# feldroop/genedex

Hardware: NVIDIA B200
Metric: len-50 count queries/s on 3.1 Gbp DNA index (locate: see `locate`) (higher is better)
Workload: dtype u64

## Files before the change

genedex_b200/_lib.py:

```python
from __future__ import annotations

import ctypes as C
import os

_HERE = os.path.dirname(os.path.abspath(__file__))
LIB_PATH = os.environ.get("GENEDEX_B200_LIB") or os.path.join(_HERE, "csrc", "libgenedex_b200.so")

GDX_OK, GDX_ERR_INVALID_SYMBOL, GDX_ERR_BAD_ARG, GDX_ERR_CUDA, GDX_ERR_OOM, GDX_ERR_TEXT_TOO_LONG, \
    GDX_ERR_UNSUPPORTED, GDX_ERR_BUSY = range(8)
GDX_I32, GDX_U32, GDX_I64 = 0, 1, 2
GDX_CONSTRUCT_HOST, GDX_CONSTRUCT_DEVICE, GDX_CONSTRUCT_AUTO = 0, 1, 2
GDX_FLAG_VERIFY_SUFFIX_ARRAY = 1
GDX_FLAG_NO_TEXT = 2
GDX_FLAG_NO_INVERSE_SAMPLES = 4
GDX_FLAG_NO_DENSE_SUFFIX_ARRAY = 8
GDX_FLAG_NO_SEED_TABLE = 16
GDX_FLAG_NO_ROW_CONTEXT_TABLE = 32
GDX_QUERIES_IO_BYTES, GDX_QUERIES_PACKED_2BIT = 0, 1
GDX_RANK_CONDENSED, GDX_RANK_FLAT = 0, 1
GDX_NCCL_UNIQUE_ID_BYTES = 128
GDX_ABI_VERSION = 2
GDX_HAMMING_MAX_MISMATCHES = 3
GDX_HAMMING_MAX_QUERY_LEN = 256

# ... 33 lines not shown
                ("lookup_table_depth", C.c_uint32), ("sampled_suffix_array_u32", C.c_void_p),
                ("flags", C.c_uint32), ("accelerator_budget_bytes", C.c_uint64),
                ("rank_variant", C.c_uint32), ("block_bits", C.c_uint32)]


class gdx_index_info(C.Structure):
    _fields_ = [("text_len", C.c_uint64), ("num_texts", C.c_uint64), ("num_dense_symbols", C.c_uint32),
                ("num_searchable_dense_symbols", C.c_uint32), ("storage", C.c_uint32),
                ("sampling_rate", C.c_uint32), ("lookup_table_depth", C.c_uint32), ("rank_layout", C.c_uint32),
                ("rank_record_bytes", C.c_uint32), ("rank_positions_per_record", C.c_uint32),
                ("device", C.c_int32), ("image_bytes", C.c_uint64), ("rank_bytes", C.c_uint64),
                ("sample_bytes", C.c_uint64), ("lookup_bytes", C.c_uint64), ("num_samples", C.c_uint64),
                ("num_text_borders", C.c_uint64), ("text_bytes", C.c_uint64),
                ("inverse_sample_bytes", C.c_uint64), ("dense_suffix_array_bytes", C.c_uint64), ("seed_table_bytes", C.c_uint64),
                ("seed_table_depth", C.c_uint32), ("row_context_entry_bytes", C.c_uint32)]


class gdx_stats(C.Structure):
    _fields_ = [("queries", C.c_uint64), ("lf_steps", C.c_uint64), ("hits", C.c_uint64),
                ("walk_steps", C.c_uint64), ("kernel_ms_search", C.c_double),
                ("kernel_ms_locate", C.c_double), ("kernel_launches", C.c_uint64),
                ("verified_queries", C.c_uint64), ("locate_walk_steps", C.c_uint64),
                ("packed_queries", C.c_uint64), ("exception_queries", C.c_uint64), ("h2d_bytes", C.c_uint64),
                ("d2h_bytes", C.c_uint64), ("shards", C.c_uint64)]


_vp, _u64, _i32, _u32 = C.c_void_p, C.c_uint64, C.c_int32, C.c_uint32
_P = C.POINTER
PROTOTYPES = {
    "gdx_abi_version": (_u32, []),
    "gdx_last_error_message": (C.c_char_p, []),
    "gdx_last_error_query": (_u64, []),
    "gdx_device_count": (_i32, []),
    "gdx_index_build": (C.c_int, [_vp, _vp, _u64, _P(gdx_alphabet), _P(gdx_config), _P(_vp)]),
    "gdx_index_create_from_parts": (C.c_int, [_P(gdx_parts), _i32, _P(_vp)]),
    "gdx_index_create_from_bwt": (C.c_int, [_vp, _P(gdx_parts), _i32, _P(_vp)]),
    "gdx_suffix_array": (C.c_int, [_vp, _u64, _u32, _u32, _i32, _vp]),
    "gdx_concat_texts": (C.c_int, [_vp, _vp, _u64, _P(gdx_alphabet), _vp, _vp, _vp]),
    "gdx_index_download_bwt": (C.c_int, [_vp, _vp]),
    "gdx_index_get_count": (C.c_int, [_vp, _vp]),
    "gdx_index_download_samples": (C.c_int, [_vp, _vp]),
    "gdx_index_download_text_borders": (C.c_int, [_vp, _vp, _vp]),
    "gdx_index_destroy": (None, [_vp]),
    "gdx_index_get_info": (C.c_int, [_vp, _P(gdx_index_info)]),
    "gdx_index_set_dense_suffix_array": (C.c_int, [_vp, C.c_int32]),
    "gdx_index_set_seed_table_depth": (C.c_int, [_vp, C.c_int32]),
    "gdx_index_set_text_verification": (C.c_int, [_vp, C.c_int32]),
# ... 63 lines not shown
```

genedex_b200/csrc/api.cu:

```cuda
#include <cuda_runtime.h>
#include <dlfcn.h>
#include <type_traits>

#include <algorithm>
#include <atomic>
#include <chrono>
#include <condition_variable>
#include <cstddef>
#include <deque>
#include <thread>
#include <cstdarg>
#include <cstdio>
#include <cstdlib>
#include <cstring>
#include <memory>
#include <mutex>
#include <shared_mutex>
#include <new>
#include <numeric>
#include <string>
#include <utility>
#include <vector>

#include <cub/device/device_radix_sort.cuh>
// ... 600 lines not shown
    if (cudaMalloc(&d, bytes) != cudaSuccess) {
        cudaGetLastError();
        return fail(GDX_ERR_OOM, "row context table: %llu bytes of device memory not available", (unsigned long long)bytes);
    }
    gdx_status st = dispatch_layout(idx->h.layout, [&](auto L) -> gdx_status {
        k_build_row_context<decltype(L)><<<(unsigned)div_up(n, 256), 256>>>(idx->dev, reinterpret_cast<uint4 *>(d), n);
        return GDX_OK;
    });
    cudaError_t e = st == GDX_OK ? cudaDeviceSynchronize() : cudaSuccess;
    if (st != GDX_OK || e != cudaSuccess) {
        cudaFree(d);
        return st != GDX_OK ? st : fail(GDX_ERR_CUDA, "row context table: %s", cudaGetErrorString(e));
    }
    idx->row_ctx = d;
    idx->row_ctx_bytes = bytes;
    idx->dev.row_context = d;
    return GDX_OK;
}

void drop_seed_table(gdx_index *idx) {
    if (!idx->seed_lut) return;
    idx->dev.seed_lookup = nullptr;
    idx->dev.seed_depth = 0;
    cudaFree(idx->seed_lut);
    idx->seed_lut = nullptr;
    idx->seed_lut_bytes = 0;
}

uint64_t seed_entries(uint32_t ns, uint32_t d) {
    uint64_t e = 1;
    for (uint32_t i = 0; i < d; ++i) {
        e *= ns;
        if (e > (1ull << 36)) return 0;
    }
    return e;
}

gdx_status build_seed_table(gdx_index *idx, uint32_t depth) {
    drop_seed_table(idx);
    const ImageHeader &h = idx->h;
    if (depth <= h.lookup_depth || h.n == 0 || h.ns == 0) return GDX_OK;
    const uint64_t esz = h.wide ? 16 : 8, last = seed_entries(h.ns, depth), prev = seed_entries(h.ns, depth - 1);
    if (last == 0 || depth > 40) return fail(GDX_ERR_UNSUPPORTED, "seed table of depth %u is too large", depth);
    void *fin = nullptr, *tmp = nullptr;
    if (cudaMalloc(&fin, last * esz) != cudaSuccess || cudaMalloc(&tmp, prev * esz) != cudaSuccess) {
        cudaGetLastError();
        if (fin) cudaFree(fin);
        return fail(GDX_ERR_OOM, "seed table of depth %u: %llu bytes of device memory not available", depth,
                    (unsigned long long)((last + prev) * esz));
    }
    void *cur = (depth % 2 == 0) ? fin : tmp;
    cudaError_t e;
    if (h.wide) {
        const uint64_t e0[2] = {0, h.n};
        e = cudaMemcpy(cur, e0, sizeof e0, cudaMemcpyHostToDevice);
    } else {
        const uint32_t e0[2] = {0, (uint32_t)h.n};
        e = cudaMemcpy(cur, e0, sizeof e0, cudaMemcpyHostToDevice);
    }
    gdx_status st = GDX_OK;
    for (uint32_t d = 1; d <= depth && e == cudaSuccess && st == GDX_OK; ++d) {
        void *nxt = cur == fin ? tmp : fin;
        const uint64_t entries = seed_entries(h.ns, d);
        st = dispatch_layout(h.layout, [&](auto L) -> gdx_status {
            k_lut_extend<decltype(L)><<<(unsigned)div_up(entries, 256), 256>>>(idx->dev, cur, nxt, entries);
            return GDX_OK;
        });
        e = cudaGetLastError();
        cur = nxt;
    }
    if (e == cudaSuccess && st == GDX_OK) e = cudaDeviceSynchronize();
    cudaFree(tmp);
    if (st != GDX_OK || e != cudaSuccess || cur != fin) {
        cudaFree(fin);
        return st != GDX_OK ? st : fail(GDX_ERR_CUDA, "seed table: %s", cudaGetErrorString(e));
    }
    idx->seed_lut = fin;
    idx->seed_lut_bytes = last * esz;
    idx->dev.seed_lookup = fin;
    idx->dev.seed_depth = depth;
    return GDX_OK;
}

uint64_t accel_room(const gdx_index *idx) {
    if (idx->h.accel_budget) {
        const uint64_t used = idx->dense_sa_bytes + idx->seed_lut_bytes + idx->row_ctx_bytes;
        return idx->h.accel_budget > used ? idx->h.accel_budget - used : 0;
    }
    size_t free_b = 0, total_b = 0;
    if (cudaMemGetInfo(&free_b, &total_b) != cudaSuccess) return 0;
    return free_b / 4;
}

void auto_seed_table(gdx_index *idx) {
    if (!idx || idx->h.n == 0 || idx->h.ns < 2) return;
    const char *e = getenv("GDX_SEED_TABLE");
    uint32_t depth = 0;
    if (e) {
        if (atoi(e) <= 0) return;
        depth = (uint32_t)atoi(e);
    } else {
        if (idx->h.accel_flags & kAccelNoSeedTable) return;
        while (seed_entries(idx->h.ns, depth + 1) && seed_entries(idx->h.ns, depth + 1) <= 4 * idx->h.n) ++depth;
        const uint64_t esz = idx->h.wide ? 16 : 8, room = accel_room(idx);
        size_t free_b = 0, total_b = 0;
        if (cudaMemGetInfo(&free_b, &total_b) != cudaSuccess) return;
        while (depth > 0 && (seed_entries(idx->h.ns, depth) * esz > room ||
                             (seed_entries(idx->h.ns, depth) + seed_entries(idx->h.ns, depth - 1)) * esz > free_b))
            --depth;
    }
    if (depth <= idx->h.lookup_depth) return;
    if (build_seed_table(idx, depth) != GDX_OK) t_error.clear();
}

void auto_dense_sa(gdx_index *idx) {
    if (!idx || idx->h.n == 0) return;
    const char *e = getenv("GDX_DENSE_SA");
    if (e && atoi(e) == 0) return;
    if (!(e && atoi(e) != 0)) {
        if (idx->h.accel_flags & kAccelNoDenseSA) return;
        if (idx->h.n * (idx->h.wide ? 8ull : 4ull) > accel_room(idx)) return;
    }
    if (build_dense_sa(idx) != GDX_OK) t_error.clear();
}

void auto_row_context(gdx_index *idx) {
    if (!idx || !row_context_possible(idx)) return;
    const char *e = getenv("GDX_ROW_CONTEXT");
    if (e && atoi(e) == 0) return;
    if (!(e && atoi(e) != 0)) {
        if (idx->h.accel_flags & kAccelNoRowContext) return;
        const uint64_t room = idx->h.accel_budget ? accel_room(idx) : 2 * accel_room(idx);
        if (idx->h.n * 16 > room) return;
    }
    if (build_row_context(idx) != GDX_OK) t_error.clear();
}

gdx_status build_image(const ImageSources &src, int device, gdx_index **out) {
    std::unique_ptr<gdx_index> idx(new gdx_index());
    GDX_TRY(plan_header(src, idx->h));
    ImageHeader &h = idx->h;
    idx->device = device;
    CUDA_TRY(cudaMalloc(&idx->image, h.image_bytes));
    idx->own_image = true;
    auto cleanup = [&](gdx_status st) {
        cudaFree(idx->image);
        idx->image = nullptr;
        return st;
    };
#define IMG_TRY(expr)                                                                             \
    do {                                                                                          \
        cudaError_t _e = (expr);                                                                  \
        if (_e != cudaSuccess)                                                                    \
            return cleanup(fail(GDX_ERR_CUDA, "%s failed: %s (%s:%d)", #expr,                     \
                                cudaGetErrorString(_e), __FILE__, __LINE__));                     \
    } while (0)
    uint8_t *base = (uint8_t *)idx->image;
    IMG_TRY(cudaMemset(base, 0, h.image_bytes));
// ... 232 lines not shown
        }
    
        if (construction == GDX_CONSTRUCT_DEVICE) {
            DeviceBuildResult r;
            const bool verify = (config->flags & GDX_FLAG_VERIFY_SUFFIX_ARRAY) != 0;
            st = device_build_from_text(nullptr, d_text.p, n, alphabet->num_dense_symbols,
                                        config->suffix_array_sampling_rate, r, t_error, false, verify, keep_isa);
            if (st != GDX_OK) return st;
            if (verify && r.verify_violations) {
                r.release();
                return fail(GDX_ERR_CUDA, "device suffix array failed verification (%llu violations)",
                            (unsigned long long)r.verify_violations);
            }
            src.border_rows = r.border_rows.data();
            src.border_pos = r.border_pos.data();
            src.n_border = r.border_rows.size();
            src.d_bwt = r.d_bwt;
            src.d_samples = r.d_samples;
            src.d_samples_wide = false;
            src.d_isa32 = r.d_isa_samples;
            st = build_image(src, device, out);
            r.release();
            if (st == GDX_OK) {
                auto_dense_sa(*out);
                auto_seed_table(*out);
                auto_row_context(*out);
            }
            return st;
        }
    
        HostParts hp;
        host_parts_from_text(ct.text.data(), n, alphabet->num_dense_symbols, config->suffix_array_sampling_rate, hp);
        uint8_t *d_bwt = nullptr;
        CUDA_TRY(cudaMalloc(&d_bwt, n ? n : 1));
        cudaError_t e = cudaMemcpy(d_bwt, hp.bwt.data(), n, cudaMemcpyHostToDevice);
        if (e != cudaSuccess) {
            cudaFree(d_bwt);
            return fail(GDX_ERR_CUDA, "BWT upload failed: %s", cudaGetErrorString(e));
        }
        src.border_rows = hp.border_rows.data();
        src.border_pos = hp.border_pos.data();
        src.n_border = hp.border_rows.size();
        src.d_bwt = d_bwt;
        src.h_samples64 = hp.samples.data();
        if (keep_isa) src.h_isa64 = hp.isa_samples.data();
        st = build_image(src, device, out);
        cudaFree(d_bwt);
        if (st == GDX_OK) {
            auto_dense_sa(*out);
            auto_seed_table(*out);
            auto_row_context(*out);
        }
        return st;
    });
}

static gdx_status sources_from_parts(const gdx_parts *parts, ImageSources &src,
                                     std::vector<uint64_t> &rows, std::vector<uint64_t> &pos) {
    if (!parts) return fail(GDX_ERR_BAD_ARG, "parts is NULL");
    GDX_TRY(validate_alphabet(parts->alphabet));
    if (parts->sampling_rate == 0) return fail(GDX_ERR_BAD_ARG, "sampling rate must be > 0");
    if (!parts->count || !parts->sentinel_indices || parts->num_texts == 0)
        return fail(GDX_ERR_BAD_ARG, "count / sentinel_indices missing");
    if (parts->text_len > storage_max(parts->storage)) return fail(GDX_ERR_TEXT_TOO_LONG, "text too long for storage");
    std::vector<std::pair<uint64_t, uint64_t>> b(parts->num_text_borders);
    for (uint64_t i = 0; i < parts->num_text_borders; ++i)
        b[i] = {parts->text_border_rows[i], parts->text_border_positions[i]};
    std::sort(b.begin(), b.end());
    rows.resize(b.size());
    pos.resize(b.size());
    for (size_t i = 0; i < b.size(); ++i) {
        rows[i] = b[i].first;
        pos[i] = b[i].second;
    }
// ... 20 lines not shown
extern "C" gdx_status gdx_index_create_from_bwt(const uint8_t *bwt, const gdx_parts *parts, int32_t device_req,
                                                gdx_index **out) {
    return guarded([&]() -> gdx_status {
        if (!out) return fail(GDX_ERR_BAD_ARG, "out is NULL");
        *out = nullptr;
        if (!bwt) return fail(GDX_ERR_BAD_ARG, "bwt is NULL");
        ImageSources src;
        std::vector<uint64_t> rows, pos;
        GDX_TRY(sources_from_parts(parts, src, rows, pos));
        int device;
        GDX_TRY(resolve_device(device_req, &device));
        DeviceGuard guard(device);
        uint8_t *d_bwt = nullptr;
        CUDA_TRY(cudaMalloc(&d_bwt, src.n ? src.n : 1));
        cudaError_t e = cudaMemcpy(d_bwt, bwt, src.n, cudaMemcpyHostToDevice);
        if (e != cudaSuccess) {
            cudaFree(d_bwt);
            return fail(GDX_ERR_CUDA, "BWT upload failed: %s", cudaGetErrorString(e));
        }
        src.d_bwt = d_bwt;
        gdx_status st = build_image(src, device, out);
        cudaFree(d_bwt);
        if (st == GDX_OK) {
            auto_dense_sa(*out);
            auto_seed_table(*out);
            auto_row_context(*out);
        }
        return st;
    });
}

extern "C" gdx_status gdx_index_create_from_parts(const gdx_parts *parts, int32_t device_req, gdx_index **out) {
    return guarded([&]() -> gdx_status {
        if (!out) return fail(GDX_ERR_BAD_ARG, "out is NULL");
        *out = nullptr;
        ImageSources src;
        std::vector<uint64_t> rows, pos;
        GDX_TRY(sources_from_parts(parts, src, rows, pos));
        if (!parts->interleaved_blocks) return fail(GDX_ERR_BAD_ARG, "interleaved_blocks is NULL");
        int device;
        GDX_TRY(resolve_device(device_req, &device));
        DeviceGuard guard(device);
        const uint32_t block_bits = parts->block_bits ? parts->block_bits : 64;
        if ((block_bits != 64 && block_bits != 512) || parts->rank_variant > GDX_RANK_FLAT)
            return fail(GDX_ERR_BAD_ARG, "rank_variant must be GDX_RANK_CONDENSED or GDX_RANK_FLAT, block_bits 64 or 512");
        const bool flat = parts->rank_variant == GDX_RANK_FLAT;
        const uint32_t words = block_bits / 64, used = block_bits - (flat ? 16 : 0);
        const uint32_t units = flat ? parts->alphabet.num_dense_symbols : choose_layout(parts->alphabet.num_dense_symbols).planes;
        const uint64_t nwords = div_up(src.n + 1, used) * units * words;
        uint64_t *d_blocks = nullptr;
        uint8_t *d_bwt = nullptr;
        CUDA_TRY(cudaMalloc(&d_blocks, nwords * 8));
        cudaError_t e = cudaMalloc(&d_bwt, src.n ? src.n : 1);
        if (e == cudaSuccess) e = cudaMemcpy(d_blocks, parts->interleaved_blocks, nwords * 8, cudaMemcpyHostToDevice);
        if (e == cudaSuccess && src.n) {
            k_ref_blocks_to_bwt<<<(unsigned)div_up(src.n, 256), 256>>>(d_blocks, flat ? 1u : 0u, words, units, src.n, d_bwt);
            e = cudaGetLastError();
        }
        cudaFree(d_blocks);
        if (e != cudaSuccess) {
            if (d_bwt) cudaFree(d_bwt);
            return fail(GDX_ERR_CUDA, "block upload failed: %s", cudaGetErrorString(e));
        }
        src.d_bwt = d_bwt;
        gdx_status st = build_image(src, device, out);
        cudaFree(d_bwt);
        if (st == GDX_OK) {
            auto_dense_sa(*out);
            auto_seed_table(*out);
            auto_row_context(*out);
        }
        return st;
    });
}

extern "C" gdx_status gdx_concat_texts(const uint8_t *texts, const uint64_t *text_offsets, uint64_t num_texts,
                                       const gdx_alphabet *alphabet, uint8_t *dense_out, uint64_t *sentinels_out,
                                       uint64_t *count_out) {
    return guarded([&]() -> gdx_status {
        if (!text_offsets || !alphabet || !dense_out || !sentinels_out || !count_out || num_texts == 0)
            return fail(GDX_ERR_BAD_ARG, "NULL argument or no texts");
        GDX_TRY(check_text_offsets(text_offsets, num_texts));
        GDX_TRY(validate_alphabet(*alphabet));
        ConcatText ct;
        uint64_t bad = 0;
        gdx_status st = concat_texts(texts, text_offsets, num_texts, *alphabet, ct, &bad);
        if (st != GDX_OK) {
            t_error_query = bad;
            return fail(st, "text %llu contains a symbol that is not in the alphabet (alphabet.rs:195-198)",
                        (unsigned long long)bad);
        }
        memcpy(dense_out, ct.text.data(), ct.text.size());
        memcpy(sentinels_out, ct.sentinels.data(), ct.sentinels.size() * 8);
// ... 240 lines not shown
                                            int32_t own_image, gdx_index **out) {
    return guarded([&]() -> gdx_status {
        if (!header || !device_image || !out) return fail(GDX_ERR_BAD_ARG, "NULL argument");
        *out = nullptr;
        ImageHeader h;
        memcpy(&h, header, sizeof h);
        GDX_TRY(validate_header(h));
        int device;
        GDX_TRY(resolve_device(device_req, &device));
        gdx_index *idx = new (std::nothrow) gdx_index();
        if (!idx) return fail(GDX_ERR_OOM, "out of host memory");
        idx->h = h;
        idx->image = device_image;
        idx->own_image = own_image != 0;
        idx->device = device;
        idx->dev = make_dev_index(h, device_image);
        {
            DeviceGuard guard(device);
            gdx_status st = init_policies(idx);
            if (st != GDX_OK) {
                delete idx;
                return st;
            }
            auto_dense_sa(idx);
            auto_seed_table(idx);
            auto_row_context(idx);
        }
        *out = idx;
        return GDX_OK;
    });
}

extern "C" gdx_status gdx_index_set_seed_table_depth(gdx_index *idx, int32_t depth) {
    return guarded([&]() -> gdx_status {
        if (!idx) return fail(GDX_ERR_BAD_ARG, "NULL argument");
        std::unique_lock<std::shared_mutex> cfg(idx->cfg_mu, std::try_to_lock);
        if (!cfg.owns_lock()) return fail(GDX_ERR_BUSY, "queries are running on this index: the seed table cannot change now");
        DeviceGuard guard(idx->device);
        if (depth <= 0) {
            drop_seed_table(idx);
            return GDX_OK;
        }
        return build_seed_table(idx, (uint32_t)depth);
    });
}

extern "C" gdx_status gdx_index_set_row_context_table(gdx_index *idx, int32_t on) {
    return guarded([&]() -> gdx_status {
        if (!idx) return fail(GDX_ERR_BAD_ARG, "NULL argument");
        std::unique_lock<std::shared_mutex> cfg(idx->cfg_mu, std::try_to_lock);
        if (!cfg.owns_lock()) return fail(GDX_ERR_BUSY, "queries are running on this index: the row context table cannot change now");
        DeviceGuard guard(idx->device);
        if (on) return build_row_context(idx);
        drop_row_context(idx);
        return GDX_OK;
    });
}

extern "C" gdx_status gdx_index_set_text_verification(gdx_index *idx, int32_t on) {
    return guarded([&]() -> gdx_status {
        if (!idx) return fail(GDX_ERR_BAD_ARG, "NULL argument");
        std::unique_lock<std::shared_mutex> cfg(idx->cfg_mu, std::try_to_lock);
        if (!cfg.owns_lock()) return fail(GDX_ERR_BUSY, "queries are running on this index");
        idx->verify = on != 0;
        return GDX_OK;
    });
// ... 760 lines not shown
        CUDA_TRY(cudaEventRecord(sl.ev_h2d, sl.stream));
        sl.h2d_pending = true;
    }
    return GDX_OK;
}

gdx_status search_result(Workspace *ws, const gdx_stats &io) {
    CUDA_TRY(ws->read_counters(ws->slot[0].stream));
    CUDA_TRY(cudaStreamSynchronize(ws->slot[0].stream));
    const Counters &cnt = *ws->cnt_h;
    t_stats.queries = io.queries;
    t_stats.packed_queries = io.packed_queries;
    t_stats.exception_queries = io.exception_queries;
    t_stats.h2d_bytes = io.h2d_bytes;
    t_stats.d2h_bytes += io.d2h_bytes;
    for (const Slot &s : ws->slot) {
        t_stats.kernel_ms_search += s.timing.elapsed_ms();
        t_stats.kernel_ms_locate += s.locate.timing.elapsed_ms();
    }
    t_stats.lf_steps = cnt.search.lf_steps;
    t_stats.walk_steps = cnt.search.verify_walk_steps + cnt.locate_walk_steps;
    t_stats.locate_walk_steps = cnt.locate_walk_steps;
    t_stats.verified_queries = cnt.search.verified_rows;
    return kernel_error(*std::min_element(cnt.err, cnt.err + kSlots),
                        "symbol in io representation should be valid (alphabet.rs:195-198)");
}

template <class Sink>
gdx_status search_host(const gdx_index *idx, Workspace *ws, const gdx_queries *qs, Sink &sink) {
    const uint64_t nq = qs->nq;
    CUDA_TRY(ws->reset_counters(ws->slot[0].stream));
    CUDA_TRY(cudaEventRecord(ws->ev_a, ws->slot[0].stream));
    for (int s = 1; s < kSlots; ++s) CUDA_TRY(cudaStreamWaitEvent(ws->slot[s].stream, ws->ev_a, 0));
    Trace trace;
    const bool prepacked = qs->encoding == GDX_QUERIES_PACKED_2BIT;
    const uint64_t total_syms = query_bytes_end(qs, nq) - query_bytes_end(qs, 0);
    const uint64_t total_in = prepacked ? (total_syms + 3) / 4 : total_syms;
    const bool pack = nq && !prepacked && idx->pack.usable && pack_enabled() && total_in >= kPackMinBytes;
    const bool src_pinned = nq && is_pinned(qs->bytes);
    Staging u{nq && total_in >= kStageMinBytes && !src_pinned,
              nq && qs->offsets && nq * 8 >= kStageMinBytes && !is_pinned(qs->offsets),
              qs->offsets && nq * 8 >= kStageMinBytes && narrow_enabled()};
    gdx::ChunkPlan plan{qs->offsets, qs->fixed_len, qs->first_symbol, nq, prepacked, pack, pack && src_pinned,
                        kChunkFirst, kChunkMax, kChunkTail, kChunkMaxQueries, 4.0e6 * HostPool::get().threads()};
    LinkQueue link;
    for (Slot &sl : ws->slot) sl.h2d_pending = false;
// ... 338 lines not shown
        HostPool::t_caller_helps = helps;
    };
    std::vector<std::thread> threads;
    threads.reserve(n_local);
    uint32_t started = 1;
    try {
        for (; started < n_local; ++started) threads.emplace_back(run, started);
    } catch (const std::exception &) {
    }
    run(0);
    for (uint32_t k = started; k < n_local; ++k) run(k);
    for (auto &t : threads) t.join();
    gdx_stats sum = {};
    gdx_status st = GDX_OK;
    for (uint32_t k = 0; k < n_local; ++k) {
        const gdx_stats &x = res[k].stats;
        sum.queries += x.queries;
        sum.lf_steps += x.lf_steps;
        sum.hits += x.hits;
        sum.walk_steps += x.walk_steps;
        sum.locate_walk_steps += x.locate_walk_steps;
        sum.kernel_launches += x.kernel_launches;
        sum.verified_queries += x.verified_queries;
        sum.packed_queries += x.packed_queries;
        sum.exception_queries += x.exception_queries;
        sum.h2d_bytes += x.h2d_bytes;
        sum.d2h_bytes += x.d2h_bytes;
        sum.kernel_ms_search = std::max(sum.kernel_ms_search, x.kernel_ms_search);
        sum.kernel_ms_locate = std::max(sum.kernel_ms_locate, x.kernel_ms_locate);
        if (st == GDX_OK && res[k].st != GDX_OK) {
            st = res[k].st;
            t_error = res[k].error;
            t_error_query = res[k].error_query;
        }
    }
    sum.shards = n_local;
    t_stats = sum;
    return st;
}

}

extern "C" gdx_status gdx_count_many_sharded(gdx_index *const *replicas, uint32_t n_local, uint32_t first_shard,
                                             uint32_t n_shards, const gdx_queries *queries, uint64_t *counts) {
    return guarded([&] {
        return run_sharded(replicas, n_local, first_shard, n_shards, queries, [&](uint32_t k, uint64_t b, uint64_t e) {
// ... 600 lines not shown
```

genedex_b200/csrc/device_index.h:

```cpp
#ifndef GDX_DEVICE_INDEX_H
#define GDX_DEVICE_INDEX_H

#include <stdint.h>

#include "rank_core.h"

namespace gdx {

constexpr uint64_t kImageMagic = 0x3130305842584447ull;
constexpr uint32_t kMaxLookupDepth = 24;
constexpr uint32_t kAccelNoDenseSA = 1, kAccelNoSeedTable = 2, kAccelNoRowContext = 4;

struct ImageHeader {
    uint64_t magic;
    uint32_t version;
    uint32_t wide;
    uint64_t n;
    uint64_t ntexts;
    uint64_t n_border;
    uint64_t n_samples;
    uint64_t n_records;
    uint64_t n_superblocks;
    uint32_t sigma, ns, storage, sampling_rate, lookup_depth;
    uint32_t accel_flags;
// ... 11 lines not shown
};

struct DevIndex {
    const uint8_t *records;
    const uint64_t *sbc;
    const void *samples;
    const void *lookup;
    const uint64_t *border_rows;
    const uint64_t *border_pos;
    const uint64_t *sentinels;
    const uint64_t *count;
    const uint8_t *text;
    const void *isa;
    const void *seed_lookup;
    const void *row_context;
    uint64_t n, ntexts, n_border;
    uint32_t sigma, ns, sampling_rate, lookup_depth;
    uint32_t wide, noff, stride, derived_symbol;
    uint32_t sampling_shift;
    uint32_t text_bits;
    uint32_t verify_min_remaining;
    uint32_t isa_rate;
    uint32_t seed_depth;
    uint64_t lut_level_off[kMaxLookupDepth + 1];
    uint64_t lut_pow[kMaxLookupDepth + 1];
    uint8_t io_to_dense[256];
};

inline DevIndex make_dev_index(const ImageHeader &h, const void *image) {
    const uint8_t *base = (const uint8_t *)image;
    DevIndex d;
    d.records = base + h.off_records;
    d.sbc = (const uint64_t *)(base + h.off_sbc);
    d.samples = base + h.off_samples;
    d.lookup = base + h.off_lookup;
    d.border_rows = (const uint64_t *)(base + h.off_border_rows);
    d.border_pos = (const uint64_t *)(base + h.off_border_pos);
    d.sentinels = (const uint64_t *)(base + h.off_sentinels);
    d.count = (const uint64_t *)(base + h.off_count);
    d.text = h.text_bits ? base + h.off_text : nullptr;
    d.text_bits = h.text_bits;
    d.isa = h.has_isa ? base + h.off_isa : nullptr;
    d.n = h.n;
    d.ntexts = h.ntexts;
    d.n_border = h.n_border;
    d.sigma = h.sigma;
    d.ns = h.ns;
    d.sampling_rate = h.sampling_rate;
    d.lookup_depth = h.lookup_depth;
    d.wide = h.wide;
    d.noff = h.layout.noff;
    d.stride = h.layout.stride;
    d.derived_symbol = h.layout.derived_symbol;
    d.sampling_shift = 0xffffffffu;
    d.verify_min_remaining = 8;
    d.isa_rate = h.sampling_rate;
    d.seed_lookup = nullptr;
    d.seed_depth = 0;
    d.row_context = nullptr;
    if ((h.sampling_rate & (h.sampling_rate - 1)) == 0) {
        uint32_t s = 0;
        while ((1u << s) < h.sampling_rate) ++s;
        d.sampling_shift = s;
    }
    for (uint32_t i = 0; i <= kMaxLookupDepth; ++i) {
        d.lut_level_off[i] = h.lut_level_off[i];
        d.lut_pow[i] = h.lut_pow[i];
    }
    for (int i = 0; i < 256; ++i) d.io_to_dense[i] = h.io_to_dense[i];
    return d;
}

}
#endif
```

genedex_b200/csrc/kernels.cuh:

```cuda
#ifndef GDX_KERNELS_CUH
#define GDX_KERNELS_CUH

#include <cuda_runtime.h>
#include <stdint.h>

#include <cub/block/block_scan.cuh>

#include "device_index.h"
#include "hamming.h"
#include "row_context.h"

namespace gdx {

struct DevQueries {
    const uint8_t *bytes;
    const uint64_t *offsets;
    const uint32_t *offsets32;
    uint64_t fixed_len;
    uint64_t nq;
    uint64_t base;
    uint64_t shift;
    const uint32_t *packed;
    uint64_t limit;
};
// ... 230 lines not shown
        const uint64_t ns = bs + L::local_rank(rs, c, s);
        e = bs + L::local_rank(rs, c, e);
        s = ns;
        return;
    }
    typename L::Rec re = L::load(ix, e, c);
    const uint64_t be = sbc_load(ix, e, c);
    s = bs + L::local_rank(rs, c, s);
    e = be + L::local_rank(re, c, e);
}

__device__ __forceinline__ void lut_load(const DevIndex &ix, uint64_t entry, uint64_t &s, uint64_t &e) {
    if (ix.wide) {
        ulonglong2 v = __ldg(reinterpret_cast<const ulonglong2 *>(ix.lookup) + entry);
        s = v.x;
        e = v.y;
    } else {
        uint2 v = __ldg(reinterpret_cast<const uint2 *>(ix.lookup) + entry);
        s = v.x;
        e = v.y;
    }
}

__device__ __forceinline__ void seed_load(const DevIndex &ix, uint64_t entry, uint64_t &s, uint64_t &e) {
    if (ix.wide) {
        const ulonglong2 v = __ldg(reinterpret_cast<const ulonglong2 *>(ix.seed_lookup) + entry);
        s = v.x;
        e = v.y;
    } else {
        const uint2 v = __ldg(reinterpret_cast<const uint2 *>(ix.seed_lookup) + entry);
        s = v.x;
        e = v.y;
    }
}

__device__ __forceinline__ void report_error(uint64_t *err, uint64_t q) {
    if (err) atomicMin(reinterpret_cast<unsigned long long *>(err), (unsigned long long)q);
}

template <class L>
__device__ __forceinline__ uint64_t resolve_row(const DevIndex &ix, uint64_t i, uint32_t &steps) {
    for (;;) {
        const bool sampled = ix.sampling_shift != 0xffffffffu ? (i & ((1ull << ix.sampling_shift) - 1)) == 0
                                                              : (i % ix.sampling_rate) == 0;
        if (sampled) {
            const uint64_t k = ix.sampling_shift != 0xffffffffu ? i >> ix.sampling_shift : i / ix.sampling_rate;
            if (ix.wide) return __ldg(reinterpret_cast<const uint64_t *>(ix.samples) + k) + steps;
            const uint32_t *sp = reinterpret_cast<const uint32_t *>(ix.samples) + k;
// ... 161 lines not shown
    }
    return key;
}

__global__ void __launch_bounds__(256)
k_query_keys(const __grid_constant__ DevIndex ix, const DevQueries qs, uint32_t key_bits, uint32_t key_syms,
             uint32_t *__restrict__ keys, uint32_t *__restrict__ idx) {
    const uint64_t q = (uint64_t)blockIdx.x * blockDim.x + threadIdx.x;
    if (q >= qs.nq) return;
    keys[q] = query_sort_key(ix, qs, q, key_bits, key_syms);
    idx[q] = (uint32_t)q;
}

constexpr uint32_t kQueryStage = 64;
constexpr uint32_t kQuerySlotWords = kQueryStage / 4 + 1;

constexpr int kModeNarrow = 8;
constexpr uint64_t kBadOffsetFlag = 1ull << 62;

struct SearchCounters {
    unsigned long long lf_steps;
    unsigned long long verify_walk_steps;
    unsigned long long verified_rows;
};

template <class L, bool VERIFY, bool CURSORS, bool PACKED>
__global__ void __launch_bounds__(256, VERIFY ? L::kVerifyMinBlocks : L::kSearchMinBlocks)
k_search(const __grid_constant__ DevIndex ix, const DevQueries qs, uint64_t *__restrict__ out_a,
         uint64_t *__restrict__ out_b, int mode_flags, uint64_t q_index_base, uint64_t *err,
         SearchCounters *stats, const uint32_t *__restrict__ perm,
         const uint32_t *__restrict__ slot_map) {
    constexpr uint32_t kTabBytes = PACKED ? 4 : 256;
    constexpr uint32_t kStageWords = PACKED ? 1 : 256 * kQuerySlotWords;
    __shared__ uint8_t tab[kTabBytes];
    __shared__ uint16_t tab2[PACKED ? 2 : 256];
    __shared__ uint32_t stage[kStageWords];
    if constexpr (!PACKED) {
        for (int i = threadIdx.x; i < 256; i += blockDim.x) {
            const uint32_t d = ix.io_to_dense[i];
            tab[i] = (uint8_t)d;
            tab2[i] = ctx_tab2_entry(d, ix.ns);
        }
        __syncthreads();
    }
    const int mode = mode_flags & 7;
    const bool narrow = (mode_flags & kModeNarrow) != 0;
// ... 46 lines not shown
        };
        auto lookup_index = [&](uint64_t p0, uint32_t d, bool &ok) -> uint64_t {
            if (coded && ix.ns == 4 && d <= 32 && p0 >= tail_begin)
                return d ? tail_bits(ptail, (uint32_t)(p0 - tail_begin), d) : 0ull;
            uint64_t li = 0, f = 1;
            for (uint32_t j = 0; j < d; ++j) {
                const uint32_t c = symbol_at(p0 + j);
                if (c == 0 || c > ix.ns) ok = false;
                li += (uint64_t)(c - 1) * f;
                f *= ix.ns;
            }
            return li;
        };

        const uint32_t depth = len < ix.lookup_depth ? (uint32_t)len : ix.lookup_depth;
        uint64_t pos = len - depth;
        uint64_t s = 0, e = 0;
        bool seeded = false;
        if (!bad && ix.seed_lookup && len >= ix.seed_depth) {
            const uint64_t p0 = len - ix.seed_depth;
            bool ok = true;
            const uint64_t li = lookup_index(p0, ix.seed_depth, ok);
            if (ok) {
                seed_load(ix, li, s, e);
                pos = p0;
                seeded = true;
            }
        }
        if (!seeded) {
            bool ok = true;
            const uint64_t li = lookup_index(pos, depth, ok);
            bad = bad || !ok || broken;
            if (!bad) lut_load(ix, ix.lut_level_off[depth] + li, s, e);
        }

        bool direct = false;
        while (!bad && pos > 0 && s != e) {
            if (VERIFY && e - s == 1 && pos >= ix.verify_min_remaining &&
                (!CURSORS || len - pos >= ix.isa_rate)) {
                uint64_t at;
                vrows = 1;
                uint64_t jm = 0;
                uint32_t cm = 0;
                int cmp = -1;
                if (!CURSORS && ix.row_context) {
                    CtxEntry en;
                    {
                        uint64_t e0, e1;
                        ldg128_na(reinterpret_cast<const uint4 *>(ix.row_context) + s, e0, e1);
                        en = CtxEntry{(uint32_t)e0, (uint32_t)(e0 >> 32), (uint32_t)e1, (uint32_t)(e1 >> 32)};
                    }
                    at = en.x;
                    if (coded && tail_begin == 0 && pos <= ctx_valid_len(en))
                        cmp = ctx_matches(en, (uint32_t)pos, ptail.lo, ptail.hi) ? 0 : 1;
                } else {
                    at = resolve_row<L>(ix, s, vsteps);
                }
                if (cmp >= 0) {
                } else if constexpr (PACKED) {
                    cmp = ix.text_bits == 4
                              ? compare_with_text<4, false>(ix, PackedQueryWords<4>{ptail, qs.packed, begin, tail_begin}, pos, at, jm, cm)
                              : compare_with_text<8, false>(ix, PackedQueryWords<8>{ptail, qs.packed, begin, tail_begin}, pos, at, jm, cm);
                } else {
                    cmp = ix.text_bits == 4
// ... 41 lines not shown
            if (mode == 0) {
                a32[slot_q] = (uint32_t)s;
                b32[slot_q] = (uint32_t)e;
            } else {
                a32[slot_q] = (uint32_t)(e - s);
            }
        } else if (mode == 0) {
            out_a[slot_q] = s;
            out_b[slot_q] = e;
        } else if (mode == 1) {
            out_a[slot_q] = e - s;
        } else {
            out_a[slot_q] = s;
            out_b[slot_q] = direct ? kDirectHit : e;
        }
    }
    if (stats) {
        uint32_t tot = __reduce_add_sync(0xffffffffu, steps);
        if ((threadIdx.x & 31) == 0 && tot) atomicAdd(&stats->lf_steps, (unsigned long long)tot);
        if (VERIFY) {
            tot = __reduce_add_sync(0xffffffffu, vsteps);
            if ((threadIdx.x & 31) == 0 && tot) atomicAdd(&stats->verify_walk_steps, (unsigned long long)tot);
            tot = __reduce_add_sync(0xffffffffu, vrows);
            if ((threadIdx.x & 31) == 0 && tot) atomicAdd(&stats->verified_rows, (unsigned long long)tot);
        }
    }
}

template <class L>
__global__ void __launch_bounds__(256)
k_extend(const __grid_constant__ DevIndex ix, uint64_t *__restrict__ starts, uint64_t *__restrict__ ends,
         const uint8_t *__restrict__ io_symbols, uint64_t n, uint64_t *err, uint64_t index_base) {
    const uint64_t q = (uint64_t)blockIdx.x * blockDim.x + threadIdx.x;
    if (q >= n) return;
    uint32_t c = ix.io_to_dense[io_symbols[q]];
    if (c == 0) {
        report_error(err, index_base + q);
        return;
    }
    uint64_t s = starts[q], e = ends[q];
    if (s > ix.n || e > ix.n) {
        report_error(err + 1, index_base + q);
        return;
    }
    if (s != e) {
        lf_pair<L>(ix, c, s, e);
        starts[q] = s;
// ... 361 lines not shown
        sbc[sb * noff + c] = acc;
        acc += t;
    }
}

template <class L>
__global__ void __launch_bounds__(256)
k_lut_fill(const __grid_constant__ DevIndex ix, void *__restrict__ lookup, uint32_t d) {
    const uint64_t i = (uint64_t)blockIdx.x * blockDim.x + threadIdx.x;
    if (i >= ix.lut_pow[d]) return;
    uint64_t s, e;
    lut_load(ix, ix.lut_level_off[d - 1] + i / ix.ns, s, e);
    const uint32_t c = (uint32_t)(i % ix.ns) + 1;
    if (s != e) lf_pair<L>(ix, c, s, e);
    const uint64_t entry = ix.lut_level_off[d] + i;
    if (ix.wide)
        reinterpret_cast<ulonglong2 *>(lookup)[entry] = make_ulonglong2(s, e);
    else
        reinterpret_cast<uint2 *>(lookup)[entry] = make_uint2((uint32_t)s, (uint32_t)e);
}

template <class L>
__global__ void __launch_bounds__(256)
k_lut_extend(const __grid_constant__ DevIndex ix, const void *__restrict__ prev, void *__restrict__ out, uint64_t entries) {
    const uint64_t i = (uint64_t)blockIdx.x * blockDim.x + threadIdx.x;
    if (i >= entries) return;
    uint64_t s, e;
    if (ix.wide) {
        const ulonglong2 v = reinterpret_cast<const ulonglong2 *>(prev)[i / ix.ns];
        s = v.x;
        e = v.y;
    } else {
        const uint2 v = reinterpret_cast<const uint2 *>(prev)[i / ix.ns];
        s = v.x;
        e = v.y;
    }
    const uint32_t c = (uint32_t)(i % ix.ns) + 1;
    if (s != e) lf_pair<L>(ix, c, s, e);
    if (ix.wide)
        reinterpret_cast<ulonglong2 *>(out)[i] = make_ulonglong2(s, e);
    else
        reinterpret_cast<uint2 *>(out)[i] = make_uint2((uint32_t)s, (uint32_t)e);
}

__global__ void k_ref_blocks_to_bwt(const uint64_t *__restrict__ blocks, uint32_t flat, uint32_t words, uint32_t units,
                                    uint64_t n, uint8_t *__restrict__ bwt) {
    const uint64_t i = (uint64_t)blockIdx.x * blockDim.x + threadIdx.x;
    if (i >= n) return;
    const uint32_t used = words * 64 - (flat ? 16 : 0);
    const uint64_t g = i / used;
    const uint32_t bit = (uint32_t)(i % used) + (flat ? 16 : 0);
    const uint64_t *grp = blocks + g * units * words + bit / 64;
    uint32_t s = 0;
    if (flat) {
        for (uint32_t c = 0; c < units; ++c)
            if ((grp[(uint64_t)c * words] >> (bit & 63)) & 1u) s = c;
    } else {
        for (uint32_t p = 0; p < units; ++p) s |= (uint32_t)((grp[(uint64_t)p * words] >> (bit & 63)) & 1u) << p;
    }
    bwt[i] = (uint8_t)s;
}

template <class L>
__global__ void __launch_bounds__(256)
k_records_to_bwt(const __grid_constant__ DevIndex ix, uint64_t begin, uint64_t end, uint8_t *__restrict__ out) {
// ... 100 lines not shown
```

genedex_b200/csrc/row_context.h:

```cpp
#ifndef GDX_ROW_CONTEXT_H
#define GDX_ROW_CONTEXT_H

#include <stdint.h>

#include "rank_core.h"

namespace gdx {

constexpr uint32_t kCtxSymbols = 45;

struct CtxEntry {
    uint32_t x, y, z, w;
};

struct PackedTail {
    uint64_t lo, hi;
};

GDX_HD uint32_t ctx_valid_len(const CtxEntry &en) { return en.w >> 26; }

template <class TextSymbol>
GDX_HD CtxEntry ctx_make_entry(uint64_t at, uint32_t ns, TextSymbol text_symbol) {
    uint32_t w0 = 0, w1 = 0, w2 = 0, vl = 0;
    for (uint32_t k = 1; k <= kCtxSymbols && k <= at; ++k) {
// ... 7 lines not shown
    }
    return CtxEntry{(uint32_t)at, w0, w1, w2 | (vl << 26)};
}

GDX_HD bool ctx_matches(const CtxEntry &en, uint32_t pos, uint64_t ql, uint64_t qh) {
    const uint64_t lo = (uint64_t)en.y | ((uint64_t)en.z << 32), hi = en.w & 0x3ffffffu;
    const uint32_t sh = 2 * (kCtxSymbols - pos);
    uint64_t rl, rh;
    if (sh == 0) {
        rl = lo;
        rh = hi;
    } else if (sh < 64) {
        rl = (lo >> sh) | (hi << (64 - sh));
        rh = hi >> sh;
    } else {
        rl = hi >> (sh - 64);
        rh = 0;
    }
    const uint32_t nb = 2 * pos;
    const uint64_t ml = nb >= 64 ? ~0ull : (1ull << nb) - 1, mh = nb > 64 ? (1ull << (nb - 64)) - 1 : 0ull;
    return (((rl ^ ql) & ml) | ((rh ^ qh) & mh)) == 0;
}

GDX_HD uint32_t bytes_at(uint32_t w0, uint32_t w1, uint32_t mis) {
#ifdef __CUDA_ARCH__
    return __byte_perm(w0, w1, 0x3210u + 0x1111u * mis);
#else
    return (uint32_t)((((uint64_t)w1 << 32) | w0) >> (8 * mis));
#endif
}

GDX_HD bool codes_from_staged(const uint16_t *tab2, const uint32_t *slot, uint32_t mis, uint32_t tail, PackedTail &t) {
    uint32_t c0 = 0, c1 = 0, c2 = 0, c3 = 0, flags = 0;
    uint32_t w0 = slot[0];
#ifdef __CUDA_ARCH__
#pragma unroll
#endif
    for (uint32_t k = 0; k < 16; ++k) {
        if (4 * k < tail) {
            const uint32_t w1 = slot[k + 1];
            const uint32_t w = bytes_at(w0, w1, mis);
            w0 = w1;
            uint32_t x = (uint32_t)tab2[w & 0xffu] + 4u * tab2[(w >> 8) & 0xffu] + 16u * tab2[(w >> 16) & 0xffu] +
                         64u * tab2[w >> 24];
            const uint32_t cnt = tail - 4 * k;
            if (cnt < 4) x &= 0x0101u * ((1u << (2 * cnt)) - 1u);
// ... 29 lines not shown
```

include/genedex_b200.h:

```cpp
#ifndef GENEDEX_B200_H
#define GENEDEX_B200_H

#include <stddef.h>
#include <stdint.h>

#ifdef __cplusplus
extern "C" {
#endif

#define GDX_ABI_VERSION 2

typedef enum gdx_status {
    GDX_OK = 0,
    GDX_ERR_INVALID_SYMBOL = 1,
    GDX_ERR_BAD_ARG = 2,
    GDX_ERR_CUDA = 3,
    GDX_ERR_OOM = 4,
    GDX_ERR_TEXT_TOO_LONG = 5,
    GDX_ERR_UNSUPPORTED = 6,
    GDX_ERR_BUSY = 7
} gdx_status;

typedef enum gdx_storage { GDX_I32 = 0, GDX_U32 = 1, GDX_I64 = 2 } gdx_storage;

// ... 94 lines not shown
    uint64_t text_bytes;
    uint64_t inverse_sample_bytes;
    uint64_t dense_suffix_array_bytes;
    uint64_t seed_table_bytes;
    uint32_t seed_table_depth;
    uint32_t row_context_entry_bytes;
} gdx_index_info;

typedef struct gdx_stats {
    uint64_t queries;
    uint64_t lf_steps;
    uint64_t hits;
    uint64_t walk_steps;
    double kernel_ms_search;
    double kernel_ms_locate;
    uint64_t kernel_launches;
    uint64_t verified_queries;
    uint64_t locate_walk_steps;
    uint64_t packed_queries;
    uint64_t exception_queries;
    uint64_t h2d_bytes;
    uint64_t d2h_bytes;
    uint64_t shards;
} gdx_stats;

uint32_t gdx_abi_version(void);
const char *gdx_last_error_message(void);
uint64_t gdx_last_error_query(void);
int32_t gdx_device_count(void);

gdx_status gdx_index_build(const uint8_t *texts, const uint64_t *text_offsets, uint64_t num_texts,
                           const gdx_alphabet *alphabet, const gdx_config *config, gdx_index **out);

gdx_status gdx_index_create_from_parts(const gdx_parts *parts, int32_t device, gdx_index **out);

gdx_status gdx_index_create_from_bwt(const uint8_t *bwt, const gdx_parts *parts, int32_t device,
                                     gdx_index **out);

gdx_status gdx_suffix_array(const uint8_t *dense_text, uint64_t n, uint32_t num_dense_symbols,
                            uint32_t where , int32_t device, uint64_t *sa_out);

gdx_status gdx_index_download_bwt(const gdx_index *idx, uint8_t *bwt_out);
gdx_status gdx_index_get_count(const gdx_index *idx, uint64_t *count_out );
gdx_status gdx_index_download_samples(const gdx_index *idx, uint64_t *samples_out);
gdx_status gdx_index_download_text_borders(const gdx_index *idx, uint64_t *rows_out, uint64_t *positions_out);

// ... 116 lines not shown
```

rust/src/gpu/ffi.rs:

```rust
#![allow(non_camel_case_types, dead_code)]
use std::os::raw::{c_char, c_void};

pub type gdx_status = i32;
pub const GDX_ABI_VERSION: u32 = 2;
pub const GDX_FLAG_VERIFY_SUFFIX_ARRAY: u32 = 1;
pub const GDX_FLAG_NO_TEXT: u32 = 2;
pub const GDX_FLAG_NO_INVERSE_SAMPLES: u32 = 4;
pub const GDX_FLAG_NO_DENSE_SUFFIX_ARRAY: u32 = 8;
pub const GDX_FLAG_NO_SEED_TABLE: u32 = 16;
pub const GDX_FLAG_NO_ROW_CONTEXT_TABLE: u32 = 32;
pub const GDX_NCCL_UNIQUE_ID_BYTES: u32 = 128;
pub const GDX_HAMMING_MAX_MISMATCHES: u32 = 3;
pub const GDX_HAMMING_MAX_QUERY_LEN: u32 = 256;
pub const GDX_OK: gdx_status = 0;
pub const GDX_ERR_INVALID_SYMBOL: gdx_status = 1;
pub const GDX_ERR_BAD_ARG: gdx_status = 2;
pub const GDX_ERR_CUDA: gdx_status = 3;
pub const GDX_ERR_OOM: gdx_status = 4;
pub const GDX_ERR_TEXT_TOO_LONG: gdx_status = 5;
pub const GDX_ERR_UNSUPPORTED: gdx_status = 6;
pub const GDX_ERR_BUSY: gdx_status = 7;
pub const GDX_I32: u32 = 0;
pub const GDX_U32: u32 = 1;
pub const GDX_I64: u32 = 2;
// ... 78 lines not shown
    pub num_text_borders: u64,
    pub text_bytes: u64,
    pub inverse_sample_bytes: u64,
    pub dense_suffix_array_bytes: u64,
    pub seed_table_bytes: u64,
    pub seed_table_depth: u32,
    pub row_context_entry_bytes: u32,
}
#[repr(C)] #[derive(Clone, Copy)] pub struct gdx_stats {
    pub queries: u64,
    pub lf_steps: u64,
    pub hits: u64,
    pub walk_steps: u64,
    pub kernel_ms_search: f64,
    pub kernel_ms_locate: f64,
    pub kernel_launches: u64,
    pub verified_queries: u64,
    pub locate_walk_steps: u64,
    pub packed_queries: u64,
    pub exception_queries: u64,
    pub h2d_bytes: u64,
    pub d2h_bytes: u64,
    pub shards: u64,
}
#[repr(C)] #[derive(Clone, Copy)] pub struct gdx_hamming_interval {
    pub start: u64,
    pub end: u64,
    pub mismatches: u32,
    pub reserved: u32,
}

extern "C" {
    pub fn gdx_abi_version() -> u32;
    pub fn gdx_last_error_message() -> *const c_char;
    pub fn gdx_last_error_query() -> u64;
    pub fn gdx_device_count() -> i32;
    pub fn gdx_index_build(texts: *const u8, text_offsets: *const u64, num_texts: u64, alphabet: *const gdx_alphabet, config: *const gdx_config, out: *mut *mut gdx_index) -> gdx_status;
    pub fn gdx_index_create_from_parts(parts: *const gdx_parts, device: i32, out: *mut *mut gdx_index) -> gdx_status;
    pub fn gdx_index_create_from_bwt(bwt: *const u8, parts: *const gdx_parts, device: i32, out: *mut *mut gdx_index) -> gdx_status;
    pub fn gdx_suffix_array(dense_text: *const u8, n: u64, num_dense_symbols: u32, r#where: u32, device: i32, sa_out: *mut u64) -> gdx_status;
    pub fn gdx_index_download_bwt(idx: *const gdx_index, bwt_out: *mut u8) -> gdx_status;
    pub fn gdx_index_get_count(idx: *const gdx_index, count_out: *mut u64) -> gdx_status;
    pub fn gdx_index_download_samples(idx: *const gdx_index, samples_out: *mut u64) -> gdx_status;
    pub fn gdx_index_download_text_borders(idx: *const gdx_index, rows_out: *mut u64, positions_out: *mut u64) -> gdx_status;
    pub fn gdx_concat_texts(texts: *const u8, text_offsets: *const u64, num_texts: u64, alphabet: *const gdx_alphabet, dense_out: *mut u8, sentinels_out: *mut u64, count_out: *mut u64) -> gdx_status;
    pub fn gdx_index_destroy(idx: *mut gdx_index);
// ... 46 lines not shown
```

Measured before the change: 12.23 billion.

## Embed row-context verification data into seed table entries for singleton intervals

The seed table's final level can now be built as 16-byte entries. For seeds whose interval holds exactly one row, the entry stores that row plus packed text context, so a count query can verify its remaining tail straight from the seed entry instead of running further LF steps or a separate row-context lookup. A new planner builds this context-enabled seed table together with the row context table when memory allows, reserving headroom for the caller. The cost is a larger seed table, an extra build kernel, and a 128-bit load per seeded query, plus a new stats counter.

```diff
diff --git a/genedex_b200/_lib.py b/genedex_b200/_lib.py
--- a/genedex_b200/_lib.py
+++ b/genedex_b200/_lib.py
@@ -79,7 +79,8 @@
                 ("kernel_ms_locate", C.c_double), ("kernel_launches", C.c_uint64),
                 ("verified_queries", C.c_uint64), ("locate_walk_steps", C.c_uint64),
                 ("packed_queries", C.c_uint64), ("exception_queries", C.c_uint64), ("h2d_bytes", C.c_uint64),
-                ("d2h_bytes", C.c_uint64), ("shards", C.c_uint64)]
+                ("d2h_bytes", C.c_uint64), ("shards", C.c_uint64),
+                ("seed_verified_queries", C.c_uint64)]
 
 
 _vp, _u64, _i32, _u32 = C.c_void_p, C.c_uint64, C.c_int32, C.c_uint32
diff --git a/genedex_b200/csrc/api.cu b/genedex_b200/csrc/api.cu
--- a/genedex_b200/csrc/api.cu
+++ b/genedex_b200/csrc/api.cu
@@ -646,6 +646,7 @@
     if (!idx->seed_lut) return;
     idx->dev.seed_lookup = nullptr;
     idx->dev.seed_depth = 0;
+    idx->dev.seed_context = 0;
     cudaFree(idx->seed_lut);
     idx->seed_lut = nullptr;
     idx->seed_lut_bytes = 0;
@@ -660,18 +661,19 @@
     return e;
 }
 
-gdx_status build_seed_table(gdx_index *idx, uint32_t depth) {
+gdx_status build_seed_table(gdx_index *idx, uint32_t depth, bool context) {
     drop_seed_table(idx);
     const ImageHeader &h = idx->h;
     if (depth <= h.lookup_depth || h.n == 0 || h.ns == 0) return GDX_OK;
     const uint64_t esz = h.wide ? 16 : 8, last = seed_entries(h.ns, depth), prev = seed_entries(h.ns, depth - 1);
     if (last == 0 || depth > 40) return fail(GDX_ERR_UNSUPPORTED, "seed table of depth %u is too large", depth);
+    const uint64_t last_bytes = last * (context ? 16 : esz);
     void *fin = nullptr, *tmp = nullptr;
-    if (cudaMalloc(&fin, last * esz) != cudaSuccess || cudaMalloc(&tmp, prev * esz) != cudaSuccess) {
+    if (cudaMalloc(&fin, last_bytes) != cudaSuccess || cudaMalloc(&tmp, prev * esz) != cudaSuccess) {
         cudaGetLastError();
         if (fin) cudaFree(fin);
         return fail(GDX_ERR_OOM, "seed table of depth %u: %llu bytes of device memory not available", depth,
-                    (unsigned long long)((last + prev) * esz));
+                    (unsigned long long)(last_bytes + prev * esz));
     }
     void *cur = (depth % 2 == 0) ? fin : tmp;
     cudaError_t e;
@@ -687,7 +689,11 @@
         void *nxt = cur == fin ? tmp : fin;
         const uint64_t entries = seed_entries(h.ns, d);
         st = dispatch_layout(h.layout, [&](auto L) -> gdx_status {
-            k_lut_extend<decltype(L)><<<(unsigned)div_up(entries, 256), 256>>>(idx->dev, cur, nxt, entries);
+            k_lut_extend<decltype(L)><<<(unsigned)div_up(entries, 256), 256>>>(idx->dev, cur, nxt, entries,
+                                                                              context && d == depth);
+            if (context && d == depth)
+                k_seed_context<decltype(L)><<<(unsigned)div_up(entries, 256), 256>>>(idx->dev, reinterpret_cast<uint4 *>(nxt),
+                                                                                    entries);
             return GDX_OK;
         });
         e = cudaGetLastError();
@@ -700,9 +706,10 @@
         return st != GDX_OK ? st : fail(GDX_ERR_CUDA, "seed table: %s", cudaGetErrorString(e));
     }
     idx->seed_lut = fin;
-    idx->seed_lut_bytes = last * esz;
+    idx->seed_lut_bytes = last_bytes;
     idx->dev.seed_lookup = fin;
     idx->dev.seed_depth = depth;
+    idx->dev.seed_context = context ? 1 : 0;
     return GDX_OK;
 }
 
@@ -714,6 +721,12 @@
     size_t free_b = 0, total_b = 0;
     if (cudaMemGetInfo(&free_b, &total_b) != cudaSuccess) return 0;
     return free_b / 4;
+}
+
+uint32_t auto_seed_depth(const gdx_index *idx) {
+    uint32_t depth = 0;
+    while (seed_entries(idx->h.ns, depth + 1) && seed_entries(idx->h.ns, depth + 1) <= 4 * idx->h.n) ++depth;
+    return depth;
 }
 
 void auto_seed_table(gdx_index *idx) {
@@ -725,7 +738,7 @@
         depth = (uint32_t)atoi(e);
     } else {
         if (idx->h.accel_flags & kAccelNoSeedTable) return;
-        while (seed_entries(idx->h.ns, depth + 1) && seed_entries(idx->h.ns, depth + 1) <= 4 * idx->h.n) ++depth;
+        depth = auto_seed_depth(idx);
         const uint64_t esz = idx->h.wide ? 16 : 8, room = accel_room(idx);
         size_t free_b = 0, total_b = 0;
         if (cudaMemGetInfo(&free_b, &total_b) != cudaSuccess) return;
@@ -734,7 +747,7 @@
             --depth;
     }
     if (depth <= idx->h.lookup_depth) return;
-    if (build_seed_table(idx, depth) != GDX_OK) t_error.clear();
+    if (build_seed_table(idx, depth, e && row_context_possible(idx)) != GDX_OK) t_error.clear();
 }
 
 void auto_dense_sa(gdx_index *idx) {
@@ -758,6 +771,33 @@
         if (idx->h.n * 16 > room) return;
     }
     if (build_row_context(idx) != GDX_OK) t_error.clear();
+}
+
+constexpr uint64_t kCallerReserve = 16ull << 30;
+
+bool context_plan(gdx_index *idx) {
+    if (!row_context_possible(idx) || getenv("GDX_SEED_TABLE") || getenv("GDX_ROW_CONTEXT") ||
+        (idx->h.accel_flags & (kAccelNoSeedTable | kAccelNoRowContext)) || idx->h.ns < 2)
+        return false;
+    const uint32_t depth = auto_seed_depth(idx);
+    if (depth <= idx->h.lookup_depth) return false;
+    size_t free_b = 0, total_b = 0;
+    if (cudaMemGetInfo(&free_b, &total_b) != cudaSuccess) return false;
+    const uint64_t seed = 16 * seed_entries(idx->h.ns, depth), fill_tmp = 8 * seed_entries(idx->h.ns, depth - 1);
+    const uint64_t room = idx->h.accel_budget ? accel_room(idx) : (free_b > kCallerReserve ? free_b - kCallerReserve : 0);
+    if (seed + 16 * idx->h.n > room || seed + fill_tmp > free_b) return false;
+    if (build_seed_table(idx, depth, true) == GDX_OK && build_row_context(idx) == GDX_OK) return true;
+    t_error.clear();
+    drop_seed_table(idx);
+    drop_row_context(idx);
+    return false;
+}
+
+void auto_accelerators(gdx_index *idx) {
+    auto_dense_sa(idx);
+    if (idx && idx->h.n && context_plan(idx)) return;
+    auto_seed_table(idx);
+    auto_row_context(idx);
 }
 
 gdx_status build_image(const ImageSources &src, int device, gdx_index **out) {
@@ -1036,9 +1076,7 @@
             st = build_image(src, device, out);
             r.release();
             if (st == GDX_OK) {
-                auto_dense_sa(*out);
-                auto_seed_table(*out);
-                auto_row_context(*out);
+                auto_accelerators(*out);
             }
             return st;
         }
@@ -1061,9 +1099,7 @@
         st = build_image(src, device, out);
         cudaFree(d_bwt);
         if (st == GDX_OK) {
-            auto_dense_sa(*out);
-            auto_seed_table(*out);
-            auto_row_context(*out);
+            auto_accelerators(*out);
         }
         return st;
     });
@@ -1130,9 +1166,7 @@
         gdx_status st = build_image(src, device, out);
         cudaFree(d_bwt);
         if (st == GDX_OK) {
-            auto_dense_sa(*out);
-            auto_seed_table(*out);
-            auto_row_context(*out);
+            auto_accelerators(*out);
         }
         return st;
     });
@@ -1174,9 +1208,7 @@
         gdx_status st = build_image(src, device, out);
         cudaFree(d_bwt);
         if (st == GDX_OK) {
-            auto_dense_sa(*out);
-            auto_seed_table(*out);
-            auto_row_context(*out);
+            auto_accelerators(*out);
         }
         return st;
     });
@@ -1463,9 +1495,7 @@
                 delete idx;
                 return st;
             }
-            auto_dense_sa(idx);
-            auto_seed_table(idx);
-            auto_row_context(idx);
+            auto_accelerators(idx);
         }
         *out = idx;
         return GDX_OK;
@@ -1482,7 +1512,7 @@
             drop_seed_table(idx);
             return GDX_OK;
         }
-        return build_seed_table(idx, (uint32_t)depth);
+        return build_seed_table(idx, (uint32_t)depth, row_context_possible(idx));
     });
 }
 
@@ -2289,6 +2319,7 @@
     t_stats.walk_steps = cnt.search.verify_walk_steps + cnt.locate_walk_steps;
     t_stats.locate_walk_steps = cnt.locate_walk_steps;
     t_stats.verified_queries = cnt.search.verified_rows;
+    t_stats.seed_verified_queries = cnt.search.seed_verified_rows;
     return kernel_error(*std::min_element(cnt.err, cnt.err + kSlots),
                         "symbol in io representation should be valid (alphabet.rs:195-198)");
 }
@@ -2673,6 +2704,7 @@
         sum.locate_walk_steps += x.locate_walk_steps;
         sum.kernel_launches += x.kernel_launches;
         sum.verified_queries += x.verified_queries;
+        sum.seed_verified_queries += x.seed_verified_queries;
         sum.packed_queries += x.packed_queries;
         sum.exception_queries += x.exception_queries;
         sum.h2d_bytes += x.h2d_bytes;
diff --git a/genedex_b200/csrc/device_index.h b/genedex_b200/csrc/device_index.h
--- a/genedex_b200/csrc/device_index.h
+++ b/genedex_b200/csrc/device_index.h
@@ -57,6 +57,7 @@
     uint32_t verify_min_remaining;
     uint32_t isa_rate;
     uint32_t seed_depth;
+    uint32_t seed_context;
     uint64_t lut_level_off[kMaxLookupDepth + 1];
     uint64_t lut_pow[kMaxLookupDepth + 1];
     uint8_t io_to_dense[256];
@@ -92,6 +93,7 @@
     d.isa_rate = h.sampling_rate;
     d.seed_lookup = nullptr;
     d.seed_depth = 0;
+    d.seed_context = 0;
     d.row_context = nullptr;
     if ((h.sampling_rate & (h.sampling_rate - 1)) == 0) {
         uint32_t s = 0;
diff --git a/genedex_b200/csrc/kernels.cuh b/genedex_b200/csrc/kernels.cuh
--- a/genedex_b200/csrc/kernels.cuh
+++ b/genedex_b200/csrc/kernels.cuh
@@ -276,8 +276,14 @@
     }
 }
 
-__device__ __forceinline__ void seed_load(const DevIndex &ix, uint64_t entry, uint64_t &s, uint64_t &e) {
-    if (ix.wide) {
+__device__ __forceinline__ void seed_load(const DevIndex &ix, uint64_t entry, uint64_t &s, uint64_t &e, CtxEntry &en) {
+    en.w = kSeedPlain << 26;
+    if (ix.seed_context) {
+        uint64_t e0, e1;
+        ldg128_na(reinterpret_cast<const uint4 *>(ix.seed_lookup) + entry, e0, e1);
+        en = CtxEntry{(uint32_t)e0, (uint32_t)(e0 >> 32), (uint32_t)e1, (uint32_t)(e1 >> 32)};
+        seed_interval(en, s, e);
+    } else if (ix.wide) {
         const ulonglong2 v = __ldg(reinterpret_cast<const ulonglong2 *>(ix.seed_lookup) + entry);
         s = v.x;
         e = v.y;
@@ -485,6 +491,7 @@
     unsigned long long lf_steps;
     unsigned long long verify_walk_steps;
     unsigned long long verified_rows;
+    unsigned long long seed_verified_rows;
 };
 
 template <class L, bool VERIFY, bool CURSORS, bool PACKED>
@@ -577,9 +584,21 @@
             bool ok = true;
             const uint64_t li = lookup_index(p0, ix.seed_depth, ok);
             if (ok) {
-                seed_load(ix, li, s, e);
+                CtxEntry en;
+                seed_load(ix, li, s, e, en);
                 pos = p0;
                 seeded = true;
+                if (VERIFY && !CURSORS && ix.row_context && seed_has_context(en) && coded && tail_begin == 0 &&
+                    pos >= ix.verify_min_remaining && pos <= ctx_valid_len(en)) {
+                    vrows = 1u << 16;
+                    if (!ctx_matches(en, (uint32_t)pos, ptail.lo, ptail.hi)) {
+                        s = e = 0;
+                        vrows |= 1u;
+                    } else if (mode != 2) {
+                        pos = 0;
+                        vrows |= 1u;
+                    }
+                }
             }
         }
         if (!seeded) {
@@ -594,7 +613,7 @@
             if (VERIFY && e - s == 1 && pos >= ix.verify_min_remaining &&
                 (!CURSORS || len - pos >= ix.isa_rate)) {
                 uint64_t at;
-                vrows = 1;
+                vrows |= 1;
                 uint64_t jm = 0;
                 uint32_t cm = 0;
                 int cmp = -1;
@@ -682,7 +701,8 @@
             tot = __reduce_add_sync(0xffffffffu, vsteps);
             if ((threadIdx.x & 31) == 0 && tot) atomicAdd(&stats->verify_walk_steps, (unsigned long long)tot);
             tot = __reduce_add_sync(0xffffffffu, vrows);
-            if ((threadIdx.x & 31) == 0 && tot) atomicAdd(&stats->verified_rows, (unsigned long long)tot);
+            if ((threadIdx.x & 31) == 0 && (tot & 0xffffu)) atomicAdd(&stats->verified_rows, (unsigned long long)(tot & 0xffffu));
+            if ((threadIdx.x & 31) == 0 && (tot >> 16)) atomicAdd(&stats->seed_verified_rows, (unsigned long long)(tot >> 16));
         }
     }
 }
@@ -1090,7 +1110,8 @@
 
 template <class L>
 __global__ void __launch_bounds__(256)
-k_lut_extend(const __grid_constant__ DevIndex ix, const void *__restrict__ prev, void *__restrict__ out, uint64_t entries) {
+k_lut_extend(const __grid_constant__ DevIndex ix, const void *__restrict__ prev, void *__restrict__ out, uint64_t entries,
+             int out_plain16) {
     const uint64_t i = (uint64_t)blockIdx.x * blockDim.x + threadIdx.x;
     if (i >= entries) return;
     uint64_t s, e;
@@ -1105,10 +1126,27 @@
     }
     const uint32_t c = (uint32_t)(i % ix.ns) + 1;
     if (s != e) lf_pair<L>(ix, c, s, e);
-    if (ix.wide)
+    if (out_plain16) {
+        const CtxEntry en = seed_plain_entry((uint32_t)s, (uint32_t)e);
+        reinterpret_cast<uint4 *>(out)[i] = make_uint4(en.x, en.y, en.z, en.w);
+    } else if (ix.wide) {
         reinterpret_cast<ulonglong2 *>(out)[i] = make_ulonglong2(s, e);
-    else
+    } else {
         reinterpret_cast<uint2 *>(out)[i] = make_uint2((uint32_t)s, (uint32_t)e);
+    }
+}
+
+template <class L>
+__global__ void __launch_bounds__(256)
+k_seed_context(const __grid_constant__ DevIndex ix, uint4 *__restrict__ table, uint64_t entries) {
+    const uint64_t i = (uint64_t)blockIdx.x * blockDim.x + threadIdx.x;
+    if (i >= entries) return;
+    const uint4 v = table[i];
+    if (v.y - v.x != 1) return;
+    uint32_t steps = 0;
+    const uint64_t at = resolve_row<L>(ix, v.x, steps);
+    const CtxEntry en = seed_context_entry(v.x, ctx_make_entry(at, ix.ns, [&](uint64_t p) { return text_symbol(ix, p); }));
+    table[i] = make_uint4(en.x, en.y, en.z, en.w);
 }
 
 __global__ void k_ref_blocks_to_bwt(const uint64_t *__restrict__ blocks, uint32_t flat, uint32_t words, uint32_t units,
diff --git a/genedex_b200/csrc/row_context.h b/genedex_b200/csrc/row_context.h
--- a/genedex_b200/csrc/row_context.h
+++ b/genedex_b200/csrc/row_context.h
@@ -53,6 +53,16 @@
     return (((rl ^ ql) & ml) | ((rh ^ qh) & mh)) == 0;
 }
 
+constexpr uint32_t kSeedPlain = 63;
+
+GDX_HD CtxEntry seed_plain_entry(uint32_t s, uint32_t e) { return CtxEntry{s, e, 0u, kSeedPlain << 26}; }
+GDX_HD CtxEntry seed_context_entry(uint32_t row, const CtxEntry &ctx) { return CtxEntry{row, ctx.y, ctx.z, ctx.w}; }
+GDX_HD bool seed_has_context(const CtxEntry &en) { return ctx_valid_len(en) != kSeedPlain; }
+GDX_HD void seed_interval(const CtxEntry &en, uint64_t &s, uint64_t &e) {
+    s = en.x;
+    e = seed_has_context(en) ? (uint64_t)en.x + 1 : (uint64_t)en.y;
+}
+
 GDX_HD uint32_t bytes_at(uint32_t w0, uint32_t w1, uint32_t mis) {
 #ifdef __CUDA_ARCH__
     return __byte_perm(w0, w1, 0x3210u + 0x1111u * mis);
diff --git a/include/genedex_b200.h b/include/genedex_b200.h
--- a/include/genedex_b200.h
+++ b/include/genedex_b200.h
@@ -140,6 +140,7 @@
     uint64_t h2d_bytes;
     uint64_t d2h_bytes;
     uint64_t shards;
+    uint64_t seed_verified_queries;
 } gdx_stats;
 
 uint32_t gdx_abi_version(void);
diff --git a/rust/src/gpu/ffi.rs b/rust/src/gpu/ffi.rs
--- a/rust/src/gpu/ffi.rs
+++ b/rust/src/gpu/ffi.rs
@@ -124,6 +124,7 @@
     pub h2d_bytes: u64,
     pub d2h_bytes: u64,
     pub shards: u64,
+    pub seed_verified_queries: u64,
 }
 #[repr(C)] #[derive(Clone, Copy)] pub struct gdx_hamming_interval {
     pub start: u64,
```

Result: slower. 9.287 billion (median of 6 runs) (-24.0%).
